# xiph/rnnoise

Hardware: AMD Instinct MI355X
Metric: 10ms frames/sec (48kHz mono) at N concurrent streams; % HBM roofline (higher is better)
Workload: dtype int8 weights x u8 activations (i32 accumulate) + f32/f64 DSP

## Files before the change

### rnnoise_amd/csrc/nn_mfma.hip

```cpp
#include "nn_common.h"
#include "dispatch.h"
#include <stdlib.h>

#define CHUNK 256
#define CH_STRIDE 260

struct MfmaLds {
  uint16_t lut[4096];
  float vadw[RN_CAT];
  union {
    struct {
      float tmp1[TS][197];
      int8_t xq[2][KT * 64 * 16];
      int8_t hq[KT * 64 * 16];
    };
    float stage[2][TS][CH_STRIDE];
  };
};

struct FrontLds {
  uint16_t lut[4096];
  float tmp1[TS][197];
  int8_t xq[2][KT * 64 * 16];
};

__device__ __forceinline__ v4i int8_tile(const int8_t *__restrict__ wmf, int rt, int lane, const int8_t *bq) {
  v4i acc = {0, 0, 0, 0};
  const v4i *a = reinterpret_cast<const v4i *>(wmf) + (size_t)rt * KT * 64 + lane;
  const v4i *b = reinterpret_cast<const v4i *>(bq) + lane;
#pragma unroll
  for (int kt = 0; kt < KT; kt++) acc = __builtin_amdgcn_mfma_i32_16x16x64_i8(a[kt * 64], b[kt * 64], acc, 0, 0, 0);
  return acc;
}

extern "C" __global__ void __launch_bounds__(NTHREADS) __attribute__((amdgpu_waves_per_eu(4)))
rn_nn_mfma_kernel(RnGroupDev g, RnModelDev m, RnTablesDev tb) {
  __shared__ __attribute__((aligned(16))) MfmaLds L;
#define RN_NN_MODE 0
#define RN_NN_LIST 1
#include "nn_tile_body.inc"
#undef RN_NN_LIST
#undef RN_NN_MODE
}
#undef NWAVES
#define NWAVES 16
extern "C" __global__ void __launch_bounds__(NTHREADS) rn_nn_mfma16_kernel(RnGroupDev g, RnModelDev m, RnTablesDev tb) {
  __shared__ __attribute__((aligned(16))) MfmaLds L;
#define RN_NN_MODE 0
#define RN_NN_LIST 1
#include "nn_tile_body.inc"
#undef RN_NN_LIST
#undef RN_NN_MODE
}
#undef NWAVES
#define NWAVES 8
extern "C" __global__ void __launch_bounds__(NTHREADS) rn_nn_front_kernel(RnGroupDev g, RnModelDev m, RnTablesDev tb) {
  __shared__ __attribute__((aligned(16))) FrontLds L;
#define RN_NN_MODE 1
#define RN_NN_LIST 0
#include "nn_tile_body.inc"
#undef RN_NN_LIST
#undef RN_NN_MODE
}
extern "C" hipError_t rn_launch_nn_mfma(const RnGroupDev *g, const RnModelDev *m, const RnTablesDev *tb, RnNnForm form, hipStream_t st,
                                        hipEvent_t e0, hipEvent_t e1) {
  if (!m->conv2.wmf || !g->nn_act || !m->dense_out.fwm || !m->conv1.fwm) return hipErrorNotSupported;
  const int n_tiles = (rn_launch_rows(g) + TS - 1) / TS;
  if (form == RN_NN_TILE16)
    RN_LAUNCH(rn_nn_mfma16_kernel, dim3(n_tiles), dim3(1024), 0, st, e0, e1, *g, *m, *tb);
  else
    RN_LAUNCH(rn_nn_mfma_kernel, dim3(n_tiles), dim3(NTHREADS), 0, st, e0, e1, *g, *m, *tb);
  return hipGetLastError();
}
extern "C" hipError_t rn_launch_nn_gru_layer(const RnGroupDev *g, const RnModelDev *m, const RnTablesDev *tb, int layer, RnGruForm form,
                                             const hipError_t lds_opt_in[2], hipStream_t st, hipEvent_t e0, hipEvent_t e1);
extern "C" hipError_t rn_launch_nn_dense(const RnGroupDev *g, const RnModelDev *m, const RnTablesDev *tb, hipStream_t st, hipEvent_t e0,
                                         hipEvent_t e1);
extern "C" hipError_t rn_launch_nn_layers(const RnGroupDev *g, const RnModelDev *m, const RnTablesDev *tb, RnGruForm gru,
                                          const hipError_t lds_opt_in[2], hipStream_t st, hipEvent_t ev[5][2]) {
  if (!m->conv2.wmf || !g->nn_act || !m->dense_out.fwm || !m->conv1.fwm || !g->act_q[0] || g->n_streams != g->n_stride) return hipErrorNotSupported;
  if ((size_t)g->n_streams * RN_GRU * 4 >= (1ull << 32)) return hipErrorNotSupported;
  const dim3 grid((g->n_streams + TS - 1) / TS);
  RN_LAUNCH(rn_nn_front_kernel, grid, dim3(NTHREADS), 0, st, ev[0][0], ev[0][1], *g, *m, *tb);
  for (int k = 0; k < 3; k++) {
    hipError_t e = rn_launch_nn_gru_layer(g, m, tb, k, gru, lds_opt_in, st, ev[1 + k][0], ev[1 + k][1]);
    if (e != hipSuccess) return e;
  }
  return rn_launch_nn_dense(g, m, tb, st, ev[4][0], ev[4][1]);
}
```

### rnnoise_amd/csrc/nn_tile_body.inc

```
  __builtin_amdgcn_s_setprio(3);
  const int tid = threadIdx.x, wave = tid >> 6, lane = tid & 63, n = lane & 15, gq = lane >> 4;
#if RN_NN_LIST
  const int N = g.list ? g.list_n : g.n_streams, s0 = blockIdx.x * TS;
#define ROW_OK(r) ((r) < N && (!g.list || (unsigned)g.list[(r)] < (unsigned)g.n_stride))
#define ROW_S(r) (g.list ? rn_list_stream_or0(g, min((r), N - 1)) : min((r), N - 1))
#else
  const int N = g.n_streams, s0 = blockIdx.x * TS;
#define ROW_OK(r) ((r) < N)
#define ROW_S(r) ((r) < N ? (r) : N - 1)
#endif
  const int sn = ROW_S(s0 + n);
  const int sil_n = g.silence[sn];
  uint32_t ownm = 0xffffu;
  if (g.model_of) {
    ownm = (uint32_t)__ballot(lane < TS && ROW_OK(s0 + lane) && rn_owns(g, ROW_S(s0 + lane)));
    if (!ownm) return;
  }
#define OWN(q) ((ownm >> (q)) & 1u)
  const bool live = ROW_OK(s0 + n) && !sil_n && OWN(n);
  const uint16_t *lut = L.lut;
#if RN_INSTRUMENT
  float *dbg = (g.debug && tid == 0) ? g.debug + (size_t)s0 * RN_DBG_FLOATS + RN_DBG_CLK2 : nullptr;
#else
  float *const dbg = nullptr;
#endif
  unsigned long long clk_prev = (RN_INSTRUMENT && g.debug) ? __builtin_amdgcn_s_memtime() : 0;
#define CLK_TAP(idx)                                           \
  do {                                                         \
    if (RN_INSTRUMENT && g.debug) {                            \
      unsigned long long now_ = __builtin_amdgcn_s_memtime();  \
      if (dbg) dbg[idx] = (float)(now_ - clk_prev);            \
      clk_prev = now_;                                         \
    }                                                          \
  } while (0)

  {
    static_assert(2048 % NTHREADS == 0, "whole trips");
    uint32_t lw[2048 / NTHREADS];
#pragma unroll
    for (int j = 0; j < 2048 / NTHREADS; j++) lw[j] = reinterpret_cast<const uint32_t *>(tb.rcp16)[tid + j * NTHREADS];
#pragma unroll
    for (int j = 0; j < 2048 / NTHREADS; j++) reinterpret_cast<uint32_t *>(L.lut)[tid + j * NTHREADS] = lw[j];
  }
#if RN_NN_MODE == 0
  {
    static_assert(RN_CAT % 512 == 0, "whole trips of the first eight waves");
    float vw_[RN_CAT / 512];
    if (NWAVES == 8 || tid < 512) {
#pragma unroll
      for (int j = 0; j < RN_CAT / 512; j++) vw_[j] = m.vad_dense.fw[tid + j * 512];
#pragma unroll
      for (int j = 0; j < RN_CAT / 512; j++) L.vadw[tid + j * 512] = vw_[j];
    }
  }
#endif
  constexpr int NE1 = (TS * 196 + NTHREADS - 1) / NTHREADS;
  float t1v[NE1];
#pragma unroll
  for (int j = 0; j < NE1; j++) {
    const int e = tid + j * NTHREADS, q = e / 196, k = e - q * 196, s = ROW_S(s0 + q);
    float v = 0;
    if (e < TS * 196 && k < 130) v = g.conv1_state[(size_t)s * 130 + k];
    else if (e < TS * 196 && k < 195) v = g.features[(size_t)s * 68 + (k - 130)];
    t1v[j] = v;
  }
  constexpr int C1WD = 4;
  const v4f *c1wq = reinterpret_cast<const v4f *>(m.conv1.fwm) + (size_t)(wave & 7) * 13 * 64 + lane;
  v4f c1w[C1WD];
#pragma unroll
  for (int u = 0; u < C1WD; u++) c1w[u] = c1wq[u * 64];
  constexpr int HC = 1024 / NTHREADS;
  v4f hist[HC];
  int hq_[HC], hk_[HC];
#pragma unroll
  for (int c = 0; c < HC; c++) {
    const int chunk = tid + c * NTHREADS, q = chunk >> 6, k = (chunk & 63) << 2;
    const int s = ROW_S(s0 + q);
    hist[c] = *reinterpret_cast<const v4f *>(g.conv2_state + (size_t)s * 256 + k);
    hq_[c] = q;
    hk_[c] = k;
    *reinterpret_cast<int *>(L.xq[0] + frag_off(q, k)) = pack4(hist[c][0], hist[c][1], hist[c][2], hist[c][3]);
  }
#pragma unroll
  for (int j = 0; j < NE1; j++) {
    const int e = tid + j * NTHREADS, q = e / 196, k = e - q * 196;
    if (e < TS * 196) L.tmp1[q][k] = t1v[j];
  }
  __syncthreads();
  constexpr int NE2 = (TS * 130 + NTHREADS - 1) / NTHREADS;
  int sil2[NE2];
#pragma unroll
  for (int j = 0; j < NE2; j++) {
    const int q = (tid + j * NTHREADS) / 130;
    sil2[j] = g.silence[ROW_S(s0 + q)];
  }
#pragma unroll
  for (int j = 0; j < NE2; j++) {
    const int e = tid + j * NTHREADS, q = e / 130, k = e - q * 130;
    if (e < TS * 130 && ROW_OK(s0 + q) && !sil2[j] && OWN(q)) g.conv1_state[(size_t)ROW_S(s0 + q) * 130 + k] = L.tmp1[q][65 + k];
  }
#pragma unroll
  for (int c = 0; c < HC; c++)
    if (hk_[c] >= 128 && ROW_OK(s0 + hq_[c]) && !g.silence[ROW_S(s0 + hq_[c])] && OWN(hq_[c]))
      *reinterpret_cast<v4f *>(g.conv2_state + (size_t)ROW_S(s0 + hq_[c]) * 256 + hk_[c] - 128) = hist[c];

  CLK_TAP(0);
  if (NWAVES == 8 || wave < 8) {
    const int rt = wave;
    v4f acc = {0, 0, 0, 0};
    const float *bx = &L.tmp1[n][gq];
#pragma unroll
    for (int u = 0; u < 12; u++) {
      const v4f a = c1w[u % C1WD];
      if (u + C1WD < 13) c1w[u % C1WD] = c1wq[(u + C1WD) * 64];
#pragma unroll
      for (int e = 0; e < 4; e++) acc = __builtin_amdgcn_mfma_f32_16x16x4f32(a[e], bx[16 * u + 4 * e], acc, 0, 0, 0);
    }
    acc = __builtin_amdgcn_mfma_f32_16x16x4f32(c1w[12 % C1WD][0], bx[192], acc, 0, 0, 0);
    const int row0 = 16 * rt + 4 * gq;
    const v4f bs = *reinterpret_cast<const v4f *>(m.conv1.bias + row0);
    v4f c1;
#pragma unroll
    for (int r = 0; r < 4; r++) c1[r] = tanh_x86(acc[r] + bs[r], lut);
    *reinterpret_cast<int *>(L.xq[0] + frag_off(n, 256 + row0)) = pack4(c1[0], c1[1], c1[2], c1[3]);
    if (live) *reinterpret_cast<v4f *>(g.conv2_state + (size_t)sn * 256 + 128 + row0) = c1;
  }
  __syncthreads();

  CLK_TAP(1);
  {
    for (int rt = wave; rt < 24; rt += NWAVES) {
      const int row0 = 16 * rt + 4 * gq;
      v4f o = int8_finish(m.conv2, row0, int8_tile(m.conv2.wmf, rt, lane, L.xq[0]));
#pragma unroll
      for (int r = 0; r < 4; r++) o[r] = tanh_x86(o[r], lut);
      if (ROW_OK(s0 + n)) *reinterpret_cast<v4f *>(g.nn_act + (size_t)sn * RN_GRU + row0) = o;
      *reinterpret_cast<int *>(L.xq[1] + frag_off(n, row0)) = pack4(o[0], o[1], o[2], o[3]);
    }
  }

#if RN_NN_MODE == 1
  __syncthreads();
  {
    v4i *dst = reinterpret_cast<v4i *>(g.act_q[0] + (size_t)blockIdx.x * (KT * 64 * 16));
    for (int i = tid; i < KT * 64; i += NTHREADS) dst[i] = reinterpret_cast<const v4i *>(L.xq[1])[i];
  }
#endif
#if RN_NN_MODE == 0
  int cur = 1;
  CLK_TAP(2);
  for (int k = 0; k < 3; k++) {
    float *st = g.gru_state + (size_t)k * g.n_stride * RN_GRU;
    for (int e = tid; e < TS * 96; e += NTHREADS) {
      const int q = e / 96, c4 = (e - q * 96) << 2, s = ROW_S(s0 + q);
      const v4f h = *reinterpret_cast<const v4f *>(st + (size_t)s * RN_GRU + c4);
      *reinterpret_cast<int *>(L.hq + frag_off(q, c4)) = pack4(h[0], h[1], h[2], h[3]);
    }
    __syncthreads();
    const RnLinearDev &wi = m.gru_in[k], &wr = m.gru_rec[k];
    for (int u = wave; u < 24; u += NWAVES) {
      const int unit0 = 16 * u + 4 * gq;
      const v4f h_old = *reinterpret_cast<const v4f *>(st + (size_t)sn * RN_GRU + unit0);
      v4f gi[3], gr[3];
#pragma unroll
      for (int gate = 0; gate < 3; gate++) {
        gi[gate] = int8_finish(wi, gate * RN_GRU + unit0, int8_tile(wi.wmf, gate * 24 + u, lane, L.xq[cur]));
        gr[gate] = int8_finish(wr, gate * RN_GRU + unit0, int8_tile(wr.wmf, gate * 24 + u, lane, L.hq));
        const v4f dg = *reinterpret_cast<const v4f *>(wr.diag + gate * RN_GRU + unit0);
#pragma unroll
        for (int r = 0; r < 4; r++) gr[gate][r] += dg[r] * h_old[r];
      }
      v4f hn;
#pragma unroll
      for (int r = 0; r < 4; r++) {
        const float z = sigmoid_x86(gi[0][r] + gr[0][r], lut);
        const float rg = sigmoid_x86(gi[1][r] + gr[1][r], lut);
        const float hh = tanh_x86(gi[2][r] + gr[2][r] * rg, lut);
        hn[r] = z * h_old[r] + (1 - z) * hh;
      }
      if (live) *reinterpret_cast<v4f *>(st + (size_t)sn * RN_GRU + unit0) = hn;
      *reinterpret_cast<int *>(L.xq[cur ^ 1] + frag_off(n, unit0)) = pack4(hn[0], hn[1], hn[2], hn[3]);
    }
    cur ^= 1;
    __syncthreads();
    CLK_TAP(3 + k);
  }
#endif
#if RN_NN_MODE == 0

  {
    const int pq = tid >> 5, pc = (tid & 31) << 2;
    const int ps = ROW_S(s0 + pq);
    auto chunk_src = [&](int c) {
      return [=](int j) {
        const int h = 2 * c + j, seg = h / 3, k0 = (h - 3 * seg) * 128;
        return *reinterpret_cast<const v4f *>((seg == 0 ? g.nn_act : g.gru_state + (size_t)(seg - 1) * g.n_stride * RN_GRU) +
                                              (size_t)ps * RN_GRU + k0 + pc);
      };
    };
    constexpr int NCH = 4 * RN_GRU / CHUNK;
    const bool prod = NWAVES == 8 || tid < 512;
    v4f park[2] = {};
    if (prod) {
      park[0] = chunk_src(0)(0);
      park[1] = chunk_src(0)(1);
      *reinterpret_cast<v4f *>(&L.stage[0][pq][pc]) = park[0];
      *reinterpret_cast<v4f *>(&L.stage[0][pq][pc + 128]) = park[1];
      park[0] = chunk_src(1)(0);
      park[1] = chunk_src(1)(1);
    }
    v4f dacc = {0, 0, 0, 0};
    float vacc = 0;
    constexpr int WDEPTH = 8, NW4 = RN_CAT / 16;
    static_assert((CHUNK / 16) % WDEPTH == 0, "a chunk is a whole number of weight-buffer rounds");
    const v4f *wq = reinterpret_cast<const v4f *>(m.dense_out.fwm) + (size_t)(wave & 1) * NW4 * 64 + lane;
    v4f wbuf[WDEPTH];
    if (wave < 2) {
#pragma unroll
      for (int u = 0; u < WDEPTH; u++) wbuf[u] = wq[u * 64];
    }
    __syncthreads();
    for (int c = 0; c < NCH; c++) {
      if (prod && c + 1 < NCH) {
        *reinterpret_cast<v4f *>(&L.stage[(c + 1) & 1][pq][pc]) = park[0];
        *reinterpret_cast<v4f *>(&L.stage[(c + 1) & 1][pq][pc + 128]) = park[1];
      }
      if (prod && c + 2 < NCH) {
        park[0] = chunk_src(c + 2)(0);
        park[1] = chunk_src(c + 2)(1);
      }
      const float(*sx)[CH_STRIDE] = L.stage[c & 1];
      if (wave < 2) {
        const float *bx = &sx[n][gq];
#pragma unroll 8
        for (int t4 = 0; t4 < CHUNK / 16; t4++) {
          const int gidx = (CHUNK / 16) * c + t4;
          const v4f a = wbuf[t4 % WDEPTH];
          if (gidx + WDEPTH < NW4) wbuf[t4 % WDEPTH] = wq[(size_t)(gidx + WDEPTH) * 64];
#pragma unroll
          for (int e = 0; e < 4; e++) dacc = __builtin_amdgcn_mfma_f32_16x16x4f32(a[e], bx[16 * t4 + 4 * e], dacc, 0, 0, 0);
        }
      } else if (wave == 2 && lane < TS) {
        const v4f *w = reinterpret_cast<const v4f *>(L.vadw + CHUNK * c);
        const v4f *x = reinterpret_cast<const v4f *>(sx[lane]);
#pragma unroll 4
        for (int j = 0; j < CHUNK / 4; j++) {
          const v4f wj = w[j], xj = x[j];
#pragma unroll
          for (int e = 0; e < 4; e++) vacc = vacc + wj[e] * xj[e];
        }
      }
      __syncthreads();
    }
    if (wave < 2) {
      const int row0 = 16 * wave + 4 * gq;
      const v4f bs = *reinterpret_cast<const v4f *>(m.dense_out.bias + row0);
      v4f o;
#pragma unroll
      for (int r = 0; r < 4; r++) o[r] = live ? sigmoid_x86(dacc[r] + bs[r], lut) : 0.f;
      if (ROW_OK(s0 + n) && OWN(n)) *reinterpret_cast<v4f *>(g.gains + (size_t)sn * RN_NB_BANDS + row0) = o;
    } else if (wave == 2 && lane < TS) {
      const int q = s0 + lane, sq = ROW_S(q);
      const bool ok = ROW_OK(q), lv = ok && !g.silence[sq];
      if (ok && OWN(lane)) g.vad[sq] = lv ? sigmoid_x86(vacc + m.vad_dense.bias[0], lut) : 0.f;
    }
  }
  CLK_TAP(6);
#endif
#undef CLK_TAP
#undef OWN
#undef ROW_OK
#undef ROW_S
```

Measured before the change: 38.53 million.

## Process two stream tiles per block in front kernel to reuse weight loads

Replaces the shared tile-body include for the front (conv1+conv2) kernel with a dedicated kernel that handles two 16-stream tiles per block. Each conv1 and conv2 weight fragment is loaded once and fed to MFMAs for both tiles, which halves weight traffic per stream and halves the grid. The quantized conv2 output is written straight to act_q from registers instead of staging through LDS and a second copy loop. In exchange the block uses more LDS and registers, which may lower occupancy.

After: 38.83 million, median of 6. About the same (+0.8%).

```diff
diff --git a/rnnoise_amd/csrc/nn_mfma.hip b/rnnoise_amd/csrc/nn_mfma.hip
--- a/rnnoise_amd/csrc/nn_mfma.hip
+++ b/rnnoise_amd/csrc/nn_mfma.hip
@@ -18,12 +18,6 @@
   };
 };
 
-struct FrontLds {
-  uint16_t lut[4096];
-  float tmp1[TS][197];
-  int8_t xq[2][KT * 64 * 16];
-};
-
 __device__ __forceinline__ v4i int8_tile(const int8_t *__restrict__ wmf, int rt, int lane, const int8_t *bq) {
   v4i acc = {0, 0, 0, 0};
   const v4i *a = reinterpret_cast<const v4i *>(wmf) + (size_t)rt * KT * 64 + lane;
@@ -54,13 +48,136 @@
 }
 #undef NWAVES
 #define NWAVES 8
+#define FT 2
+struct FrontLds {
+  uint16_t lut[4096];
+  float tmp1[FT][TS][197];
+  int8_t xq[FT][KT * 64 * 16];
+};
 extern "C" __global__ void __launch_bounds__(NTHREADS) rn_nn_front_kernel(RnGroupDev g, RnModelDev m, RnTablesDev tb) {
   __shared__ __attribute__((aligned(16))) FrontLds L;
-#define RN_NN_MODE 1
-#define RN_NN_LIST 0
-#include "nn_tile_body.inc"
-#undef RN_NN_LIST
-#undef RN_NN_MODE
+  const int tid = threadIdx.x, wave = tid >> 6, lane = tid & 63, n = lane & 15, gq = lane >> 4;
+  const int N = g.n_streams, s0 = blockIdx.x * (FT * TS);
+#define ROW_OK(r) ((r) < N)
+#define ROW_S(r) ((r) < N ? (r) : N - 1)
+  uint32_t ownm = 0xffffffffu;
+  if (g.model_of) ownm = (uint32_t)__ballot(lane < FT * TS && ROW_OK(s0 + lane) && rn_owns(g, ROW_S(s0 + lane)));
+  bool tile_ok[FT];
+#pragma unroll
+  for (int T = 0; T < FT; T++) tile_ok[T] = s0 + T * TS < N && ((ownm >> (T * TS)) & 0xffffu);
+  if (!tile_ok[0] && !tile_ok[1]) return;
+  const uint16_t *lut = L.lut;
+
+  {
+    uint32_t lw[2048 / NTHREADS];
+#pragma unroll
+    for (int j = 0; j < 2048 / NTHREADS; j++) lw[j] = reinterpret_cast<const uint32_t *>(tb.rcp16)[tid + j * NTHREADS];
+#pragma unroll
+    for (int j = 0; j < 2048 / NTHREADS; j++) reinterpret_cast<uint32_t *>(L.lut)[tid + j * NTHREADS] = lw[j];
+  }
+  constexpr int NE1 = (FT * TS * 196 + NTHREADS - 1) / NTHREADS;
+  float t1v[NE1];
+#pragma unroll
+  for (int j = 0; j < NE1; j++) {
+    const int e = tid + j * NTHREADS, q = e / 196, k = e - q * 196, s = ROW_S(s0 + q);
+    float v = 0;
+    if (e < FT * TS * 196 && k < 130) v = g.conv1_state[(unsigned)(s * 130 + k)];
+    else if (e < FT * TS * 196 && k < 195) v = g.features[(unsigned)(s * 68 + k - 130)];
+    t1v[j] = v;
+  }
+  constexpr int C1WD = 4;
+  const v4f *c1wq = reinterpret_cast<const v4f *>(m.conv1.fwm) + (size_t)wave * 13 * 64 + lane;
+  v4f c1w[C1WD];
+#pragma unroll
+  for (int u = 0; u < C1WD; u++) c1w[u] = c1wq[u * 64];
+  constexpr int HC = FT * 1024 / NTHREADS;
+  v4f hist[HC];
+#pragma unroll
+  for (int c = 0; c < HC; c++) {
+    const int chunk = tid + c * NTHREADS, q = chunk >> 6, k = (chunk & 63) << 2;
+    hist[c] = *reinterpret_cast<const v4f *>(g.conv2_state + (unsigned)(ROW_S(s0 + q) * 256 + k));
+  }
+  const uint32_t livem = ownm & (uint32_t)__ballot(lane < FT * TS && ROW_OK(s0 + lane) && !g.silence[ROW_S(s0 + lane)]);
+#define LIVE(q) ((livem >> (q)) & 1u)
+#pragma unroll
+  for (int c = 0; c < HC; c++) {
+    const int chunk = tid + c * NTHREADS, q = chunk >> 6, k = (chunk & 63) << 2;
+    *reinterpret_cast<int *>(L.xq[q >> 4] + frag_off(q & 15, k)) = pack4(hist[c][0], hist[c][1], hist[c][2], hist[c][3]);
+  }
+#pragma unroll
+  for (int j = 0; j < NE1; j++) {
+    const int e = tid + j * NTHREADS, q = e / 196, k = e - q * 196;
+    if (e < FT * TS * 196) L.tmp1[q >> 4][q & 15][k] = t1v[j];
+  }
+  __syncthreads();
+#pragma unroll
+  for (int j = 0; j < NE1; j++) {
+    const int e = tid + j * NTHREADS, q = e / 196, k = e - q * 196;
+    if (e < FT * TS * 196 && k >= 65 && k < 195 && LIVE(q)) g.conv1_state[(size_t)(s0 + q) * 130 + k - 65] = t1v[j];
+  }
+#pragma unroll
+  for (int c = 0; c < HC; c++) {
+    const int chunk = tid + c * NTHREADS, q = chunk >> 6, k = (chunk & 63) << 2;
+    if (k >= 128 && LIVE(q)) *reinterpret_cast<v4f *>(g.conv2_state + (size_t)(s0 + q) * 256 + k - 128) = hist[c];
+  }
+
+  {
+    const int rt = wave;
+    v4f acc[FT];
+#pragma unroll
+    for (int T = 0; T < FT; T++) acc[T] = v4f{0, 0, 0, 0};
+#pragma unroll
+    for (int u = 0; u < 12; u++) {
+      const v4f a = c1w[u % C1WD];
+      if (u + C1WD < 13) c1w[u % C1WD] = c1wq[(u + C1WD) * 64];
+#pragma unroll
+      for (int e = 0; e < 4; e++)
+#pragma unroll
+        for (int T = 0; T < FT; T++) acc[T] = __builtin_amdgcn_mfma_f32_16x16x4f32(a[e], L.tmp1[T][n][gq + 16 * u + 4 * e], acc[T], 0, 0, 0);
+    }
+#pragma unroll
+    for (int T = 0; T < FT; T++)
+      acc[T] = __builtin_amdgcn_mfma_f32_16x16x4f32(c1w[12 % C1WD][0], L.tmp1[T][n][gq + 192], acc[T], 0, 0, 0);
+    const int row0 = 16 * rt + 4 * gq;
+    const v4f bs = *reinterpret_cast<const v4f *>(m.conv1.bias + row0);
+#pragma unroll
+    for (int T = 0; T < FT; T++) {
+      v4f c1;
+#pragma unroll
+      for (int r = 0; r < 4; r++) c1[r] = tanh_x86(acc[T][r] + bs[r], lut);
+      *reinterpret_cast<int *>(L.xq[T] + frag_off(n, 256 + row0)) = pack4(c1[0], c1[1], c1[2], c1[3]);
+      if (LIVE(T * TS + n)) *reinterpret_cast<v4f *>(g.conv2_state + (size_t)(s0 + T * TS + n) * 256 + 128 + row0) = c1;
+    }
+  }
+  __syncthreads();
+
+  for (int rt = wave; rt < 24; rt += NWAVES) {
+    const int row0 = 16 * rt + 4 * gq;
+    const v4i *a = reinterpret_cast<const v4i *>(m.conv2.wmf) + (size_t)rt * KT * 64 + lane;
+    v4i acc[FT];
+#pragma unroll
+    for (int T = 0; T < FT; T++) acc[T] = v4i{0, 0, 0, 0};
+#pragma unroll
+    for (int kt = 0; kt < KT; kt++) {
+      const v4i ak = a[kt * 64];
+#pragma unroll
+      for (int T = 0; T < FT; T++)
+        acc[T] = __builtin_amdgcn_mfma_i32_16x16x64_i8(ak, reinterpret_cast<const v4i *>(L.xq[T])[kt * 64 + lane], acc[T], 0, 0, 0);
+    }
+#pragma unroll
+    for (int T = 0; T < FT; T++) {
+      if (!tile_ok[T]) continue;
+      v4f o = int8_finish(m.conv2, row0, acc[T]);
+#pragma unroll
+      for (int r = 0; r < 4; r++) o[r] = tanh_x86(o[r], lut);
+      const int r_ = s0 + T * TS + n;
+      if (ROW_OK(r_)) *reinterpret_cast<v4f *>(g.nn_act + (size_t)r_ * RN_GRU + row0) = o;
+      *reinterpret_cast<int *>(g.act_q[0] + (size_t)(blockIdx.x * FT + T) * (KT * 64 * 16) + frag_off(n, row0)) = pack4(o[0], o[1], o[2], o[3]);
+    }
+  }
+#undef LIVE
+#undef ROW_OK
+#undef ROW_S
 }
 extern "C" hipError_t rn_launch_nn_mfma(const RnGroupDev *g, const RnModelDev *m, const RnTablesDev *tb, RnNnForm form, hipStream_t st,
                                         hipEvent_t e0, hipEvent_t e1) {
@@ -80,7 +197,7 @@
                                           const hipError_t lds_opt_in[2], hipStream_t st, hipEvent_t ev[5][2]) {
   if (!m->conv2.wmf || !g->nn_act || !m->dense_out.fwm || !m->conv1.fwm || !g->act_q[0] || g->n_streams != g->n_stride) return hipErrorNotSupported;
   if ((size_t)g->n_streams * RN_GRU * 4 >= (1ull << 32)) return hipErrorNotSupported;
-  const dim3 grid((g->n_streams + TS - 1) / TS);
+  const dim3 grid((g->n_streams + FT * TS - 1) / (FT * TS));
   RN_LAUNCH(rn_nn_front_kernel, grid, dim3(NTHREADS), 0, st, ev[0][0], ev[0][1], *g, *m, *tb);
   for (int k = 0; k < 3; k++) {
     hipError_t e = rn_launch_nn_gru_layer(g, m, tb, k, gru, lds_opt_in, st, ev[1 + k][0], ev[1 + k][1]);
diff --git a/rnnoise_amd/csrc/nn_tile_body.inc b/rnnoise_amd/csrc/nn_tile_body.inc
--- a/rnnoise_amd/csrc/nn_tile_body.inc
+++ b/rnnoise_amd/csrc/nn_tile_body.inc
@@ -139,13 +139,6 @@
     }
   }
 
-#if RN_NN_MODE == 1
-  __syncthreads();
-  {
-    v4i *dst = reinterpret_cast<v4i *>(g.act_q[0] + (size_t)blockIdx.x * (KT * 64 * 16));
-    for (int i = tid; i < KT * 64; i += NTHREADS) dst[i] = reinterpret_cast<const v4i *>(L.xq[1])[i];
-  }
-#endif
 #if RN_NN_MODE == 0
   int cur = 1;
   CLK_TAP(2);
```
